# dyustc/CTC-Attention-Mispronunciation

Measured on AMD Instinct MI355X. Metric: phoneme-frames/sec joint CTC-attn decode, 41-phone vocab, higher is better.
Workload: dtype f32 -- reference width (operands with all 24 significand bits, fp32 accumulate; see `accuracy`: closer to a float64 evaluation than ATen's own fp32): the large time-batched contractions (conv0/conv1, BiLSTM and text input projections) run on the bf16 matrix cores as f32x6 = each fp32 operand as thre

## Files before the change

### ctc-attention-mispronunciation_amd/csrc/api.hip

```cpp
#include <stdarg.h>
#include <stdio.h>
#include <string.h>

#include <algorithm>
#include <cmath>
#include <memory>
#include <mutex>
#include <vector>

#include "mdd_internal.h"

namespace mdd {

static thread_local char g_err[512] = "";

void set_error(const char *fmt, ...) {
    va_list ap;
    va_start(ap, fmt);
    vsnprintf(g_err, sizeof(g_err), fmt, ap);
    va_end(ap);
}

struct DeviceGate {
    std::mutex mu;
// ... 266 lines not shown
    const ForwardPlan &p = m->plan;
    a.gx = m->gx.p; a.whh = lw.whh; a.hbuf = m->hbuf.p; a.cbuf = m->cbuf.p;
    a.H = m->cfg.hidden; a.packed = packed_whh(m->cfg);
    a.whh_split = lw.whh_s; a.hsplit = p.lstm == Lstm::StepX3 ? reinterpret_cast<unsigned short *>(m->hsplit.p) : nullptr;
    if (!p.gated) return launch_lstm_layer(a, st);
    info->launches = 1;
    unsigned short *hx = reinterpret_cast<unsigned short *>(m->hx.p);
    long long *stamps = m->sw.lstm_dbg && a.T > 100 ? reinterpret_cast<long long *>(m->hx.p + p.stamps_at) : nullptr;
    if (p.lstm == Lstm::X6) return launch_lstm_layer_x6(a, lw.whh_3, hx, m->sync_words.p, m->err_flag.p, st, stamps, m->sw.x6_redo_mask);
    if (p.lstm == Lstm::Granule) return launch_lstm_layer_granule(a, hx, m->sync_words.p, m->err_flag.p, st, stamps, m->sw.lstm_early);
    return launch_lstm_layer_f32(a, hx, m->sync_words.p, m->err_flag.p, st, stamps);
}

static int run_stage(mdd_model *m, int si, const float *x, int B, int T, const int64_t *x1, int L, float *logp,
                     hipStream_t st, Stage *info) {
    const mdd_config &c = m->cfg;
    const DecodeWeights &w = *m->weights;
    const int H = c.hidden, H2 = 2 * H, G2 = 8 * H, Tp = T / 2, Lp = L, nl = c.layers;
    const ForwardPlan &p = m->plan;
    const bool x3 = p.precision == 1, fused = p.conv != Conv::Separate;
    const size_t rows = (size_t)Tp * B, trows = (size_t)L * B;
    static thread_local char namebuf[32];
    Stage dummy; if (!info) info = &dummy;
    info->launches = 1; info->flops = 0.0;
    if (si == 0 && fused) {
        info->name = "conv_fused";
        info->flops = 2.0 * 9 * c.channels * (double)B * Tp * m->W2() * (c.channels + 6.0);
        if (p.conv == Conv::FusedX3)
            return launch_conv_fused(x, w.w_conv0, w.sc0, w.sh0, w.w_conv1_s, w.sc1, w.sh1, split_view(m->seq0_s, rows * m->rnn_in()),
                                     nullptr, B, T, m->raw_T, st);
        return launch_conv_fused3(x, w.w_conv0, w.sc0, w.sh0, w.w_conv1_3, w.sc1, w.sh1, reinterpret_cast<unsigned short *>(m->p3.p),
                                  m->taps ? m->seq0.p : nullptr, B, T, m->raw_T, st, p.conv == Conv::FusedX6Rowwise);
    }
    if (si == 1 && fused) { info->name = "conv1_in_fused"; info->launches = 0; return MDD_OK; }
    if (si == 0) { info->name = "conv0"; info->flops = 2.0 * 9 * c.channels * (double)B * T * m->W1();
        return launch_conv0(x, w.w_conv0, w.sc0, w.sh0, m->y0.p, B, T, c.feat, c.channels, st); }
    if (si == 1) { info->name = "conv1"; info->flops = 2.0 * 9 * c.channels * c.channels * (double)B * Tp * m->W2();
        return launch_conv1(m->y0.p, w.w_conv1t, w.sc1, w.sh1, x3 ? nullptr : m->seq0.p,
                            x3 ? split_view(m->seq0_s, rows * m->rnn_in()) : kNoSplit, B, T, m->W1(), c.channels, st); }
    si -= 2;
    if (si < 2 * nl) {
        const int n = si / 2;
        const int K = n == 0 ? m->rnn_in() : H2;
        if (si % 2 == 0) {
            snprintf(namebuf, sizeof(namebuf), "gemm_ih%d", n); info->name = namebuf;
            info->flops = 2.0 * (double)Tp * B * G2 * K;
            if (p.proj == Gemm::Bf16x3) {
                const SplitPtr in = n == 0 ? split_view(m->seq0_s, rows * K) : split_view(m->act_s[(n - 1) & 1], rows * K);
                return launch_gemm_bf16x3(in, w.rnn[n].wih_s, nullptr, m->gx.p, nullptr, Tp * B, G2, K, K, K, G2, 1, 0, 0, 0, st);
            }
            const float *in = n == 0 ? m->seq0.p : m->act[(n - 1) & 1].p;
            if (p.proj == Gemm::F32x6) {
                unsigned short *p3 = reinterpret_cast<unsigned short *>(m->p3.p);
                if (!(n == 0 && fused))
                    if (int rc = launch_split3(in, Tp * B, K, K, p3, st)) return rc;
                return launch_gemm_f32x6(p3, (size_t)Tp * B * K, w.rnn[n].wih_3, (size_t)G2 * K, nullptr, m->gx.p, Tp * B, G2, K, G2, st);
            }
            return launch_gemm_nt(in, w.rnn[n].wih, nullptr, m->gx.p, Tp * B, G2, K, K, K, G2, 1, 0, 0, 0, st);
        }
        snprintf(namebuf, sizeof(namebuf), "lstm%d", n); info->name = namebuf;
        info->launches = Tp; info->flops = 2.0 * 2 * (double)B * H * 4 * H * Tp;
        LstmStepArgs a;
        a.T = Tp; a.B = B; a.seqlen = m->tlen;
        if (n == nl - 1) {
            a.out = m->xraw.p; a.out_raw = m->xraw.p; a.oscale = nullptr; a.oshift = nullptr;
            a.out_split = x3 ? split_view(m->x_s, rows * H2) : kNoSplit;
        } else {
            a.out = x3 ? nullptr : m->act[n & 1].p; a.out_raw = m->taps ? m->tap_rnn[n].p : nullptr;
            a.out_split = x3 ? split_view(m->act_s[n & 1], rows * H2) : kNoSplit;
            a.oscale = w.rnn[n + 1].scale; a.oshift = w.rnn[n + 1].shift;
        }
        return run_lstm(m, w.rnn[n], a, st, info);
    }
    si -= 2 * nl;
    const LstmWeights &tw = w.rnn[nl];
    switch (si) {
    case 0:
        info->name = "embed";
        return launch_embed(w.emb, c.emb_rows, c.emb_dim, x1, B, L, x3 ? nullptr : m->embo.p,
                            x3 ? split_view(m->embo_s, trows * c.emb_dim) : kNoSplit, m->err_flag.p, st);
    case 1:
        info->name = "gemm_text"; info->flops = 2.0 * (double)L * B * G2 * c.emb_dim;
        if (p.proj == Gemm::Bf16x3) return launch_gemm_bf16x3(split_view(m->embo_s, trows * c.emb_dim), tw.wih_s, w.t_bias, m->gx.p, nullptr, L * B, G2,
                                                              c.emb_dim, c.emb_dim, c.emb_dim, G2, 1, 0, 0, 0, st);
        if (p.proj == Gemm::F32x6) {
            unsigned short *p3 = reinterpret_cast<unsigned short *>(m->p3.p);
            if (int rc = launch_split3(m->embo.p, L * B, c.emb_dim, c.emb_dim, p3, st)) return rc;
            return launch_gemm_f32x6(p3, (size_t)L * B * c.emb_dim, tw.wih_3, (size_t)G2 * c.emb_dim, w.t_bias, m->gx.p, L * B, G2, c.emb_dim, G2, st);
        }
        return launch_gemm_nt(m->embo.p, tw.wih, w.t_bias, m->gx.p, L * B, G2, c.emb_dim, c.emb_dim, c.emb_dim, G2, 1, 0, 0, 0, st);
    case 2: {
        info->name = "lstm_text"; info->launches = L; info->flops = 2.0 * 2 * (double)B * H * 4 * H * L;
        LstmStepArgs a;
        a.T = L; a.B = B; a.seqlen = m->llen;
        a.out = m->text.p; a.out_raw = m->text.p; a.oscale = nullptr; a.oshift = nullptr;
        a.out_split = x3 ? split_view(m->text_s, trows * H2) : kNoSplit;
        return run_lstm(m, tw, a, st, info);
    }
    case 3:
        info->name = "gemm_key"; info->flops = 2.0 * (double)L * B * H2 * H2;
        if (x3) {
            const SplitPtr ks = split_view(m->key_s, trows * H2);
            return launch_gemm_bf16x3(split_view(m->text_s, trows * H2), w.w_score_s, nullptr, nullptr, &ks, L * B, H2, H2, H2, H2, H2,
                                      1, 0, 0, 0, st);
        }
        return launch_gemm_nt(m->text.p, w.w_score, nullptr, m->key.p, L * B, H2, H2, H2, H2, H2, 1, 0, 0, 0, st);
    case 4:
        info->name = "gemm_score"; info->flops = 2.0 * (double)B * Tp * L * H2;
        if (x3) return launch_gemm_bf16x3(split_view(m->x_s, rows * H2), split_view(m->key_s, trows * H2), nullptr, m->S.p, nullptr, Tp, L,
                                          H2, B * H2, B * H2, Lp, B, H2, H2, (long)Tp * Lp, st);
        return launch_gemm_nt(m->xraw.p, m->key.p, nullptr, m->S.p, Tp, L, H2, B * H2, B * H2, Lp, B, H2, H2, (long)Tp * Lp, st);
    default:
        info->name = "attn_tail"; info->flops = 2.0 * (double)B * Tp * ((double)L * H2 + 2.0 * H2 * c.num_class);
        return launch_attn_tail(m->S.p, Lp, m->xraw.p, m->text.p, w.fscale, w.fshift, w.w_fc, w.w_fcp, logp, Tp, B, L, H2, c.num_class, st, m->llen);
    }
}

int device_gate_enter(int device, hipStream_t st, bool *held) {
    *held = false;
    hipStreamCaptureStatus cs = hipStreamCaptureStatusNone;
    if (st && hipStreamIsCapturing(st, &cs) == hipSuccess && cs != hipStreamCaptureStatusNone) return MDD_OK;
// ... 355 lines not shown
```

### ctc-attention-mispronunciation_amd/csrc/lstm_x6.hip

```cpp
#include "lstm_persist.h"
#include <type_traits>
#include <utility>

namespace mdd {

typedef __bf16 bf16x8 __attribute__((ext_vector_type(8)));

#define XSTAMP(i) do { if (DBG) { long long n_ = __builtin_readcyclecounter(); ph[i] += n_ - tst; tst = n_; } } while (0)

template <int N, typename F>
__device__ __forceinline__ void x6_static_for(F &&f) {
    if constexpr (N > 0) { x6_static_for<N - 1>(f); f(std::integral_constant<int, N - 1>{}); }
}

struct X6Args {
    const float *gx;
    const unsigned short *whh3;
    unsigned short *hx;
    unsigned int *sync;
    int *err_flag;
    float *out, *out_raw;
    const float *oscale, *oshift;
    int T, B, BGr;
    int force_mask;
    long long *dbg;
    const int *seqlen;
};

template <int H, int NBT, bool DBG = false>
__global__ __launch_bounds__(256, 1) void lstm_layer_x6_kernel(X6Args a) {
    extern __shared__ __attribute__((aligned(16))) unsigned char smem[];
    constexpr int NTH = 256, KS = H / 32, KH = KS / 2, RM = 4 * H / 16, NRT = RM / 16, UW = RM / 4;
    static_assert(NRT == 6 || NRT == 4, "H = 384 (six row tiles per member) or H = 256 (four)");
    constexpr int NT = NRT / 2;
    constexpr int CPM = UW / 8;
    constexpr bool SKEW = NBT >= 3;
    constexpr int CC = H / 8;
    constexpr int PLB = CC * 256;
    constexpr int PANB = 3 * PLB;
    constexpr int NLD = PANB / (NTH * 16);
    static_assert(PANB % (NTH * 16) == 0 && (NLD == 9 || NLD == 6), "a panel is whole passes of the workgroup");
    constexpr int NGB = NBT == 1 ? 2 : 1;
    constexpr int GXT = 16 * UW * 4;
    float *Os = reinterpret_cast<float *>(smem);
    float *Or = Os + 16 * UW;
    unsigned short *Og = reinterpret_cast<unsigned short *>(Or + 16 * UW);
    float *Gx = reinterpret_cast<float *>(Og + 3 * 3 * 16 * 8);
    unsigned char *Rw = reinterpret_cast<unsigned char *>(Gx + NBT * NGB * GXT);
    float *Px = reinterpret_cast<float *>(Rw + 2 * PANB);
    __shared__ int s_flag[3];
    const int tid = threadIdx.x, lane = tid & 63, wave = tid >> 6;
    const int li = lane & 15, kq = lane >> 4;
    const int w = blockIdx.x, xl = w & 7, jw = w >> 3;
    const int team = xl * 2 + (jw >> 4), member = jw & 15;
    const int d = team >> 3, g = team & 7;
    const int B = a.B, T = a.T;
    if (tid < 3) s_flag[tid] = 0;
    const int rh = wave >> 1, kh = wave & 1;

    bf16x8 wf[NT][KH][3];
#pragma unroll
    for (int t = 0; t < NT; t++) {
        const int rt = t < 2 ? rh * 2 + t : 4 + rh;
        const int row = member * RM + rt * 16 + li;
#pragma unroll
        for (int p = 0; p < 3; p++) {
            const unsigned short *wp = a.whh3 + ((size_t)(p * 2 + d) * 4 * H + row) * H + kq * 8 + kh * KH * 32;
#pragma unroll
            for (int j = 0; j < KH; j++) wf[t][j][p] = *reinterpret_cast<const bf16x8 *>(wp + j * 32);
        }
    }
    const int ot0 = kh == 0 ? rh * 2 : 4;
    const int widx = kh == 0 ? rh : 2;
    float osc[2], osh[2];
    const bool scaled = a.oscale != nullptr;
#pragma unroll
    for (int r = 0; r < 2; r++) {
        const int unit = member * UW + min(ot0 + r, NRT - 1) * 4 + kq;
        osc[r] = scaled ? a.oscale[d * H + unit] : 1.f;
        osh[r] = scaled ? a.oshift[d * H + unit] : 0.f;
    }
    float cst[2][NBT];
#pragma unroll
    for (int r = 0; r < 2; r++)
#pragma unroll
        for (int bt = 0; bt < NBT; bt++) cst[r][bt] = 0.f;
    int slen[NBT];
#pragma unroll
    for (int bt = 0; bt < NBT; bt++) {
        const int lb = bt * 16 + li, row = g * a.BGr + lb;
        slen[bt] = (a.seqlen && lb < a.BGr && row < B) ? a.seqlen[row] : T;
    }
    constexpr size_t tbytes = PANB;
    const size_t pbytes = (size_t)NBT * tbytes;
    unsigned char *hxb = reinterpret_cast<unsigned char *>(a.hx);
    unsigned int *abortf = a.sync + 16;
    long long ph[6] = {0, 0, 0, 0, 0, 0}, tst = DBG ? (long long)__builtin_readcyclecounter() : 0;

    const unsigned gx_lds = (unsigned)(unsigned long long)(lds_void_t *)Gx, rw_lds = (unsigned)(unsigned long long)(lds_void_t *)Rw;
// ... 29 lines not shown
#undef X6_G
#undef X6_G2
    };
    const unsigned char *const hx_team = hxb + (size_t)team * pbytes;
    auto hx_parity = [&](int sp) { return hx_team + (size_t)(sp & 1) * 16 * pbytes; };
    auto tag_word = [](int sp) -> unsigned { const unsigned ep = (unsigned)(sp % 3 + 1); return ((ep & 1u) << 14) | ((ep >> 1) << 30); };
    auto panel_stale = [&](int pb, int sp) -> bool {
        const unsigned e = tag_word(sp);
        unsigned bad = 0;
#pragma unroll
        for (int i = 0; i < NLD; i++) bad |= *reinterpret_cast<const unsigned *>(Rw + (size_t)pb * PANB + (size_t)(i * NTH + tid) * 16) ^ e;
        return (bad & 0x40004000u) != 0;
    };
    int fk = 0;
    auto wg_any = [&](bool v) -> bool {
        if (__any(v) && lane == 0) s_flag[fk] = 1;
        lds_barrier();
        const bool r = s_flag[fk] != 0;
        const int nx = fk == 2 ? 0 : fk + 1, n2 = nx == 2 ? 0 : nx + 1;
        if (tid == 0) s_flag[n2] = 0;
        fk = nx;
        return r;
    };
    int vslot = 0;
    auto post = [&](bool v) { if (__any(v) && lane == 0) s_flag[fk] = 1; };
    auto posted = [&] {
        vslot = fk;
        const int nx = fk == 2 ? 0 : fk + 1, n2 = nx == 2 ? 0 : nx + 1;
        if (tid == 0) s_flag[n2] = 0;
        fk = nx;
    };
    auto ensure_fresh = [&](int bt, int sp, int pb) -> bool {
        long long t0 = 0;
        int polls = 0;
        bool ok = true;
        for (;;) {
            request_sweep(hx_parity(sp), bt, pb);
            asm volatile("s_waitcnt vmcnt(0)" ::: "memory");
            lds_barrier();
            if ((++polls & 63) == 0) {
                bool giveup = false;
                if (t0 == 0) t0 = wall_clock64();
                if (tid == 0 && ((__hip_atomic_load(abortf, __ATOMIC_RELAXED, __HIP_MEMORY_SCOPE_AGENT) != 0) || (wall_clock64() - t0 > 200000000ll))) {
                    __hip_atomic_store(abortf, 1u, __ATOMIC_RELAXED, __HIP_MEMORY_SCOPE_AGENT); atomicExch(a.err_flag, 2); giveup = true;
                }
                if (wg_any(giveup)) { ok = false; break; }
            }
            if (!wg_any(panel_stale(pb, sp))) break;
        }
        if (DBG) ph[5] += polls;
        return ok;
    };
    const size_t slab = (size_t)B * 2 * H;
    const bool two_out = a.out_raw && a.out && a.out_raw != a.out;
    float *const out_main = a.out ? a.out : a.out_raw;
    auto tile_rows = [&](int bt) { const int nv = min(a.BGr, B - g * a.BGr) - bt * 16; return nv < 0 ? 0 : (nv > 16 ? 16 : nv); };

    auto products = [&](auto chk_, int pb, unsigned e, f32x4 *gsum, auto &&at_ks, auto &&pre) -> bool {
        constexpr bool CHK = decltype(chk_)::value;
        const unsigned char *fb = Rw + (size_t)pb * PANB + kq * 256 + li * 16 + kh * (KH * 1024);
        unsigned orall = 0u, andall = ~0u;
        if (CHK) {
            const unsigned char *ob = Rw + (size_t)pb * PANB + kq * 256 + li * 16 + (kh ^ 1) * (KH * 1024);
#pragma unroll
            for (int j = 0; j < KH; j++)
#pragma unroll
                for (int p = 0; p < 3; p++) { const unsigned v = *reinterpret_cast<const unsigned *>(ob + p * PLB + j * 1024); orall |= v; andall &= v; }
        }
        const f32x4 z = (f32x4){0.f, 0.f, 0.f, 0.f};
        f32x4 hh[NT], sm[NT];
#pragma unroll
        for (int t = 0; t < NT; t++) { hh[t] = z; sm[t] = z; }
        u32x4 fh[3][3];
#pragma unroll
        for (int p = 0; p < 3; p++) { fh[0][p] = *reinterpret_cast<const u32x4 *>(fb + p * PLB); fh[1][p] = *reinterpret_cast<const u32x4 *>(fb + p * PLB + 1024); }
        pre();
#pragma unroll
        for (int p = 0; p < 3; p++) {
            if (CHK) { orall |= fh[0][p][0]; andall &= fh[0][p][0]; }
            fh[0][p][0] &= 0xbfffbfffu;
        }
#pragma unroll
        for (int j = 0; j < KH; j++) {
            __builtin_amdgcn_sched_barrier(0x406);
            if (j + 2 < KH) {
#pragma unroll
                for (int p = 0; p < 3; p++) fh[(j + 2) % 3][p] = *reinterpret_cast<const u32x4 *>(fb + p * PLB + (j + 2) * 1024);
            }
            at_ks(j);
            if (j + 1 < KH) {
#pragma unroll
                for (int p = 0; p < 3; p++) {
                    if (CHK) { orall |= fh[(j + 1) % 3][p][0]; andall &= fh[(j + 1) % 3][p][0]; }
                    fh[(j + 1) % 3][p][0] &= 0xbfffbfffu;
                }
            }
            const bf16x8 bh = __builtin_bit_cast(bf16x8, fh[j % 3][0]), bm = __builtin_bit_cast(bf16x8, fh[j % 3][1]), bl = __builtin_bit_cast(bf16x8, fh[j % 3][2]);
#define X6_MF(acc, wp, bp) _Pragma("unroll") for (int t = 0; t < NT; t++) acc[t] = __builtin_amdgcn_mfma_f32_16x16x32_bf16(wf[t][j][wp], bp, acc[t], 0, 0, 0)
            X6_MF(sm, 1, bm); X6_MF(sm, 0, bl); X6_MF(sm, 2, bh); X6_MF(hh, 0, bh); X6_MF(sm, 0, bm); X6_MF(sm, 1, bh);
#undef X6_MF
        }
#pragma unroll
        for (int t = 0; t < NT; t++) gsum[t] = hh[t] + sm[t];
        return CHK && (((orall ^ e) | (andall ^ e)) & 0x40004000u) != 0;
    };
    auto px_at = [&](int buf, int tile, int half) -> float * { return Px + ((buf * 6 + tile) * 2 + half) * 256 + lane * 4; };
    auto send_partials = [&](auto role_, const f32x4 *gsum, int buf) {
        constexpr int ROLE = decltype(role_)::value;
#pragma unroll
        for (int t = 0; t < NT; t++) {
            const bool own = ROLE == 0 ? t < 2 : (ROLE == 1 && t == 2);
            if (!own) *reinterpret_cast<f32x4 *>(px_at(buf, t < 2 ? rh * 2 + t : 4 + rh, kh)) = gsum[t];
        }
    };

    auto cell1 = [&](auto role_, const f32x4 *gsum, int buf, auto bt_, int sc, bool on) {
        constexpr int ROLE = decltype(role_)::value;
        constexpr int bt = decltype(bt_)::value;
        const int t = d ? (T - 1 - sc) : sc;
        const unsigned tg = (unsigned)(sc % 3 + 1);
        const int lb = bt * 16 + li;
        const bool valid = lb < a.BGr && g * a.BGr + lb < B;
        const int gb = NBT == 1 ? (sc & 1) : 0;
#pragma unroll
        for (int r = 0; r < 2; r++) {
            const int rt = ot0 + r;
            f32x4 acc;
            if (ROLE == 0) acc = gsum[r] + *reinterpret_cast<const f32x4 *>(px_at(buf, rt, 1));
            else if (r == 0) acc = gsum[2] + *reinterpret_cast<const f32x4 *>(px_at(buf, 4, 0));
            else acc = *reinterpret_cast<const f32x4 *>(px_at(buf, 5, 0)) + *reinterpret_cast<const f32x4 *>(px_at(buf, 5, 1));
            const float4 gv = *reinterpret_cast<const float4 *>(Gx + (bt * NGB + gb) * GXT + (rt * 64 + lane) * 4);
            const float gi = acc[0] + gv.x, gf = acc[1] + gv.y, gg = acc[2] + gv.z, go = acc[3] + gv.w;
            const float ig = gate_sigmoid(gi), fg = gate_sigmoid(gf), cg = gate_tanh(gg), og = gate_sigmoid(go);
            const bool live = !(d && t >= slen[bt]);
            const float cn = fg * cst[r][bt] + ig * cg;
            const float hr_ = og * gate_tanh(cn);
            const float hn = (valid && live) ? hr_ : 0.f;
            cst[r][bt] = on ? (live ? cn : 0.f) : cst[r][bt];
            const int ul = rt * 4 + kq;
            Os[li * UW + ul] = scaled ? hn * osc[r] + osh[r] : hn;
            Or[li * UW + ul] = hn;
            const unsigned tagw = r == 0 ? ((kq == 0 ? (tg & 1u) : kq == 1 ? (tg >> 1) : 0u) << 14) : 0u;
            const float hs = (hn != hn) ? 1.5f : hn;
            const __bf16 b0 = (__bf16)hs;
            const float r1 = hs - (float)b0;
            const __bf16 b1 = (__bf16)r1, b2 = (__bf16)(r1 - (float)b1);
            unsigned short *og_ = Og + widx * (3 * 16 * 8) + li * 8 + r * 4 + kq;
            og_[0] = (unsigned short)(__builtin_bit_cast(unsigned short, b0) | tagw);
            og_[16 * 8] = (unsigned short)(__builtin_bit_cast(unsigned short, b1) | tagw);
            og_[2 * 16 * 8] = (unsigned short)(__builtin_bit_cast(unsigned short, b2) | tagw);
        }
    };
    auto cell2 = [&](auto bt_, const float *gxn, unsigned char *hxpub, float *outp, float *rawp, bool on) {
        constexpr int bt = decltype(bt_)::value;
        if (NBT >= 2) load_gx(bt, 0, gxn);
        {
            const int prow = lane & 15, pp = lane >> 4;
            const __amdgpu_buffer_rsrc_t drs = __builtin_amdgcn_make_buffer_rsrc(hxpub + (size_t)bt * tbytes, 0, (int)tbytes, 0x00020000);
            const u32x4 pv = *reinterpret_cast<const u32x4 *>(Og + widx * (3 * 16 * 8) + ((pp < 3 ? pp : 0) * 16 + prow) * 8);
            const unsigned off = (pp < 3 && on) ? (unsigned)(pp * PLB + ((member * CPM + (ot0 >> 1)) * 16 + prow) * 16) : 0xffffffffu;
            __builtin_amdgcn_raw_buffer_store_b128(pv, drs, off, 0, 16 );
        }
        {
            const int nr = tile_rows(bt);
            const int rr = min(lane & 15, max(nr - 1, 0)), piece = lane >> 4;
            const bool mine = piece < 2 && nr > 0 && on;
            const int rt = ot0 + (piece & 1);
            const unsigned el = (unsigned)((g * a.BGr + bt * 16 + rr) * 2 * H + d * H + member * UW + rt * 4);
            const int lo = rr * UW + rt * 4;
            const u32x4 v = *reinterpret_cast<const u32x4 *>(Os + lo);
            const __amdgpu_buffer_rsrc_t rs_ = __builtin_amdgcn_make_buffer_rsrc(outp, 0, (int)(slab * 4), 0x00020000);
            __builtin_amdgcn_raw_buffer_store_b128(v, rs_, mine ? el * 4u : 0xffffffffu, 0, 0);
            const u32x4 v2 = *reinterpret_cast<const u32x4 *>(Or + lo);
            const __amdgpu_buffer_rsrc_t rs2 = __builtin_amdgcn_make_buffer_rsrc(rawp, 0, (int)(slab * 4), 0x00020000);
            __builtin_amdgcn_raw_buffer_store_b128(v2, rs2, (mine && two_out) ? el * 4u : 0xffffffffu, 0, 0);
        }
    };

    auto run = [&](auto role_) {
        constexpr int ROLE = decltype(role_)::value;
        constexpr bool OWNER = ROLE == 0 || (ROLE == 1 && NRT == 6);
        const std::integral_constant<bool, ROLE == 2> chk_{};
#pragma unroll
        for (int i = 0; i < 2 * NLD; i++) *reinterpret_cast<u32x4 *>(Rw + (size_t)(i * NTH + tid) * 16) = (u32x4){0u, 0u, 0u, 0u};
        if constexpr (OWNER) x6_static_for<NBT>([&](auto bt_) { load_gx(decltype(bt_)::value, 0, gx_at(d ? (T - 1) : 0)); });
        asm volatile("s_waitcnt vmcnt(0)" ::: "memory");
        lds_barrier();
        f32x4 gP[NT];
#pragma unroll
        for (int t = 0; t < NT; t++) gP[t] = (f32x4){0.f, 0.f, 0.f, 0.f};
        int pc = 0;
        bool dead = false, have_v = false;
        auto redo = [&](int btv, int sv, int pbv, int pxb) {
            asm volatile("s_waitcnt vmcnt(0)" ::: "memory");
            if (!ensure_fresh(btv, sv - 1, pbv)) { dead = true; return; }
            products(std::false_type{}, pbv, 0u, gP, [](int) {}, [] {});
            send_partials(role_, gP, pxb);
            lds_barrier();
            if (DBG) ph[5] += 1000;
        };
        float *const raw_main = two_out ? a.out_raw : out_main;
        auto t_of = [&](int st) { return d ? (T - 1 - st) : st; };
        for (int s = 0; s < T && !dead; s++) {
            const int sp_ = max(s - 1, 0), sn_ = min(s + 1, T - 1);
            const float *const gx_s = gx_at(t_of(s)), *const gx_n = gx_at(t_of(sn_));
            float *const out_s = out_main + (size_t)t_of(s) * slab, *const out_p = out_main + (size_t)t_of(sp_) * slab;
            float *const raw_s = raw_main + (size_t)t_of(s) * slab, *const raw_p = raw_main + (size_t)t_of(sp_) * slab;
            unsigned char *const hx_s = const_cast<unsigned char *>(hx_parity(s)), *const hx_p = const_cast<unsigned char *>(hx_parity(s - 1));
            auto phase = [&](auto bt_) {
                constexpr int bt = decltype(bt_)::value;
                constexpr int nbt = bt + 1 < NBT ? bt + 1 : 0, pbt = bt > 0 ? bt - 1 : NBT - 1;
                const int ns = bt + 1 < NBT ? s : s + 1, psv = bt > 0 ? s : s - 1;
                const int pb = pc & 1;
                ++pc;
                f32x4 gs[NT];
                if (NBT == 1) {
                    if (s >= 1) {
                        asm volatile("s_waitcnt vmcnt(0)" ::: "memory");
                        if (!ensure_fresh(bt, s - 1, pb)) { dead = true; return; }
                    }
                    XSTAMP(0);
                    products(std::false_type{}, pb, 0u, gs, [&](int j) { if (OWNER && j == 0) load_gx(bt, (s + 1) & 1, gx_n); }, [] {});
                    XSTAMP(1);
                    send_partials(role_, gs, 0);
                    asm volatile("s_waitcnt vmcnt(0)" ::: "memory");
                    lds_barrier();
                    XSTAMP(2);
                    if constexpr (OWNER) { cell1(role_, gs, 0, bt_, s, true); XSTAMP(3); cell2(bt_, gx_n, hx_s, out_s, raw_s, true); }
                    XSTAMP(4);
                    return;
                }
                constexpr int RQJ = SKEW ? 0 : KH - 1;
                const bool stale = products(chk_, pb, tag_word(s + 2), gs, [&](int j) {
                    if (j == RQJ) request_sweep(hx_parity(ns - 1), nbt, pb ^ 1);
                    if constexpr (SKEW && OWNER) {
                        if (j == 0) cell1(role_, gP, (pc & 1), std::integral_constant<int, pbt>{}, max(psv, 0), psv >= 0);
                        if (j == 1) { if (bt > 0) cell2(std::integral_constant<int, pbt>{}, gx_n, hx_s, out_s, raw_s, true); else cell2(std::integral_constant<int, pbt>{}, gx_s, hx_p, out_p, raw_p, psv >= 0); }
                    }
                }, [&] {
                    if constexpr (SKEW) { if (have_v && s_flag[vslot] != 0) redo(pbt, psv, pb ^ 1, pc & 1); }
                }) && s >= 1;
                const bool forced = a.force_mask >= 0 && s >= 1 && (pc & a.force_mask) == 0;
                XSTAMP(1);
                send_partials(role_, gs, (pc & 1) ^ 1);
                if constexpr (SKEW) {
                    post(stale || forced);
                    if constexpr (OWNER) wait_vmcnt(3); else asm volatile("s_waitcnt vmcnt(0)" ::: "memory");
                    lds_barrier();
                    posted();
                    have_v = true;
                    XSTAMP(2);
                } else {
                    const bool again = wg_any(stale || forced);
                    XSTAMP(2);
                    if (again) {
                        asm volatile("s_waitcnt vmcnt(0)" ::: "memory");
                        if (!ensure_fresh(bt, s - 1, pb)) { dead = true; return; }
                        products(std::false_type{}, pb, 0u, gs, [](int) {}, [] {});
                        send_partials(role_, gs, (pc & 1) ^ 1);
                        lds_barrier();
                        if (DBG) ph[5] += 1000;
                    }
                }
                if (SKEW) {
#pragma unroll
                    for (int t = 0; t < NT; t++) gP[t] = gs[t];
                } else {
                    if constexpr (OWNER) cell1(role_, gs, (pc & 1) ^ 1, bt_, s, true);
                    XSTAMP(3);
                    asm volatile("s_waitcnt vmcnt(0)" ::: "memory");
                    lds_barrier();
                    if constexpr (OWNER) cell2(bt_, gx_n, hx_s, out_s, raw_s, true);
                    XSTAMP(4);
                }
                XSTAMP(0);
            };
            x6_static_for<NBT>([&](auto bt_) { if (!dead) phase(bt_); });
        }
        if constexpr (SKEW) {
            if (!dead && have_v && s_flag[vslot] != 0) redo(NBT - 1, T - 1, (pc & 1) ^ 1, (pc & 1) ^ 1);
            if constexpr (OWNER) {
                if (!dead) {
                    cell1(role_, gP, (pc & 1) ^ 1, std::integral_constant<int, NBT - 1>{}, T - 1, true);
                    cell2(std::integral_constant<int, NBT - 1>{}, gx_at(t_of(T - 1)), const_cast<unsigned char *>(hx_parity(T - 1)), out_main + (size_t)t_of(T - 1) * slab, raw_main + (size_t)t_of(T - 1) * slab, true);
                }
            }
        }
    };
    if (kh == 0) run(std::integral_constant<int, 0>{});
    else if (rh == 0) run(std::integral_constant<int, 1>{});
    else run(std::integral_constant<int, 2>{});
    if (DBG && tid == ((blockIdx.x >> 3) & 3) * 64)
        for (int i = 0; i < 6; i++) a.dbg[blockIdx.x * 6 + i] = ph[i];
}

static size_t x6_smem(int H, int NBT) {
    const int UW = H / 16;
    return (size_t)16 * UW * 4 * 2 + (size_t)3 * 3 * 16 * 8 * 2 + (size_t)NBT * (NBT == 1 ? 2 : 1) * 16 * UW * 16 + (size_t)2 * 3 * (H / 8) * 256 + (size_t)2 * 6 * 2 * 1024;
}

template <int H, int NBT, bool DBG = false>
static int launch_x6_t(const X6Args &a, hipStream_t st) {
    if (int rc = launch_zero_fill(a.sync, 32 * sizeof(unsigned int), st)) return rc;
    if (int rc = launch_zero_fill(a.hx, (size_t)2 * 16 * NBT * 3 * (H / 8) * 256, st)) return rc;
    hipLaunchKernelGGL((lstm_layer_x6_kernel<H, NBT, DBG>), dim3(kPersistGrid), dim3(256), x6_smem(H, NBT), st, a);
    MDD_LAUNCH_CHECK();
    return MDD_OK;
}

template <int H, int N>
static constexpr bool x6_built() {
#ifdef MDD_X6_DEV
    return H == 384 && N <= 4;
#else
    return true;
#endif
}
template <int H, int N>
static int launch_x6_pick(const X6Args &a, hipStream_t st) {
    if constexpr (!x6_built<H, N>()) { set_error("persistent x6 lstm: H=%d with %d tiles per team is not in this development build", H, N); return MDD_ERR_ARG; }
    else {
        if constexpr (H == 384) { if (a.dbg) return launch_x6_t<H, N, true>(a, st); }
        return launch_x6_t<H, N>(a, st);
    }
}

int launch_lstm_layer_x6(const LstmStepArgs &s, const unsigned short *whh3, unsigned short *hx, unsigned int *sync, int *err_flag, hipStream_t st,
                         long long *stamps, int force_mask) {
    X6Args a;
    a.gx = s.gx; a.whh3 = whh3; a.hx = hx; a.sync = sync; a.err_flag = err_flag;
    a.out = s.out; a.out_raw = s.out_raw; a.oscale = s.oscale; a.oshift = s.oscale ? s.oshift : nullptr;
    a.T = s.T; a.B = s.B; a.BGr = (s.B + 7) / 8; a.seqlen = s.seqlen;
    a.force_mask = force_mask;
    const int nbt = (a.BGr + 15) / 16;
    a.dbg = stamps;
    if (s.out_split.hi || s.gates_save || (!a.out && !a.out_raw) || !whh3) { set_error("persistent x6 lstm: fp32 outputs, inference only"); return MDD_ERR_ARG; }
    if (nbt < 1 || nbt > 8) { set_error("persistent x6 lstm: B=%d needs %d row tiles per team (max 8)", s.B, nbt); return MDD_ERR_ARG; }
#define X6_CASE(H_, N_) case N_: return launch_x6_pick<H_, N_>(a, st)
    if (s.H == 384) switch (nbt) { X6_CASE(384, 1); X6_CASE(384, 2); X6_CASE(384, 3); X6_CASE(384, 4); X6_CASE(384, 5); X6_CASE(384, 6); X6_CASE(384, 7); X6_CASE(384, 8); }
    if (s.H == 256) switch (nbt) { X6_CASE(256, 1); X6_CASE(256, 2); X6_CASE(256, 3); X6_CASE(256, 4); X6_CASE(256, 5); X6_CASE(256, 6); X6_CASE(256, 7); X6_CASE(256, 8); }
#undef X6_CASE
    set_error("persistent x6 lstm: unsupported H=%d", s.H);
    return MDD_ERR_ARG;
}

template <int H, int N>
static int x6_attr() {
    if constexpr (x6_built<H, N>()) {
        MDD_HIP_CHECK(hipFuncSetAttribute((const void *)lstm_layer_x6_kernel<H, N>, hipFuncAttributeMaxDynamicSharedMemorySize, 156 * 1024));
        if constexpr (H == 384) MDD_HIP_CHECK(hipFuncSetAttribute((const void *)lstm_layer_x6_kernel<H, N, true>, hipFuncAttributeMaxDynamicSharedMemorySize, 156 * 1024));
    }
    return MDD_OK;
}

int init_lstm_x6_attributes() {
#define XATTR(H, N) if (int rc = x6_attr<H, N>()) return rc
    XATTR(384, 1); XATTR(384, 2); XATTR(384, 3); XATTR(384, 4); XATTR(384, 5); XATTR(384, 6); XATTR(384, 7); XATTR(384, 8);
    XATTR(256, 1); XATTR(256, 2); XATTR(256, 3); XATTR(256, 4); XATTR(256, 5); XATTR(256, 6); XATTR(256, 7); XATTR(256, 8);
#undef XATTR
    return MDD_OK;
}

int persistent_x6_grid_fits(int n_cu) {
    if (n_cu < kPersistGrid) return 0;
    int per_cu = 0;
    constexpr int N = x6_built<384, 8>() ? 8 : 4;
    if (hipOccupancyMaxActiveBlocksPerMultiprocessor(&per_cu, (const void *)lstm_layer_x6_kernel<384, N>, 256, x6_smem(384, N)) != hipSuccess) return 0;
    return per_cu >= 1 ? 1 : 0;
}

}
```

### ctc-attention-mispronunciation_amd/csrc/mdd_internal.h

```cpp
#pragma once
#include <hip/hip_runtime.h>
#include <stdint.h>

#include <map>
#include <string>
#include <utility>
#include <vector>

#include "../../include/mdd_hip.h"
#include "plan.h"

namespace mdd {

void set_error(const char *fmt, ...);

#define MDD_HIP_CHECK(expr)                                                                     \
    do {                                                                                        \
        hipError_t e_ = (expr);                                                                 \
        if (e_ != hipSuccess) {                                                                 \
            mdd::set_error("%s failed: %s (%s:%d)", #expr, hipGetErrorString(e_), __FILE__, __LINE__); \
            return MDD_ERR_HIP;                                                                 \
        }                                                                                       \
    } while (0)

// ... 19 lines not shown
    }
};
using DeviceBuf = DeviceArray<float>;

struct SplitPtr { unsigned short *hi, *lo; };

int launch_gemm_nt(const float *A, const float *W, const float *bias, float *C, int M, int N, int K, int lda, int ldw,
                   int ldc, int batch, long sA, long sW, long sC, hipStream_t st);

int launch_gemm_f32(bool ta, bool tb, const float *A, const float *B, const float *bias, float *C, int M, int N, int K, int lda, int ldb,
                    int ldc, int batch, long sA, long sB, long sC, bool accumulate, hipStream_t st, int ksplit = 0);

int launch_gemm_bf16x3(const SplitPtr &A, const SplitPtr &W, const float *bias, float *C, const SplitPtr *Csplit, int M, int N,
                       int K, int lda, int ldw, int ldc, int batch, long sA, long sW, long sC, hipStream_t st);
int init_gemm_attributes();
int launch_split(const float *x, size_t n, const SplitPtr &out, hipStream_t st);
int launch_unsplit(const SplitPtr &in, size_t n, float *x, hipStream_t st);
int launch_split3(const float *x, int rows, int K, int ld, unsigned short *planes, hipStream_t st);
int launch_gemm_f32x6(const unsigned short *A3, size_t a_plane, const unsigned short *W3, size_t w_plane, const float *bias, float *C, int M, int N, int K,
                      int ldc, hipStream_t st, long long *stamps = nullptr);
int init_gemm_x6_attributes();

int launch_stack_skip(const float *raw, int B, int T_raw, int D, int right, int skip, int n_down, float *out,
                      hipStream_t st);
int launch_conv0(const float *x, const float *w, const float *scale, const float *shift, float *y0, int B, int T, int F,
                 int ch, hipStream_t st);
int launch_conv1(const float *y0, const float *w_t, const float *scale, const float *shift, float *seq, SplitPtr seq_split, int B,
                 int T, int W1, int ch, hipStream_t st);

int launch_conv_fused(const float *x, const float *w0, const float *sc0, const float *sh0, SplitPtr w1, const float *sc1,
                      const float *sh1, SplitPtr out, float *out_f32, int B, int T, int Traw, hipStream_t st);
int launch_conv_fused3(const float *x, const float *w0, const float *sc0, const float *sh0, const unsigned short *w1_3, const float *sc1,
                       const float *sh1, unsigned short *out3, float *out_f32, int B, int T, int Traw, hipStream_t st,
                       bool rowwise = false);
int init_conv_attributes();

struct LstmStepArgs {
    const float *gx;
    const float *whh;
    float *hbuf;
    float *cbuf;
    float *out;
    SplitPtr out_split;
    float *out_raw;
    const float *oscale;
    const float *oshift;
    int T, B, H;
    SplitPtr whh_split;
    unsigned short *hsplit;
    int packed;
    float *gates_save = nullptr;
    float *c_save = nullptr;
    const int *seqlen = nullptr;
};
int launch_lstm_layer(const LstmStepArgs &a, hipStream_t st);

int launch_embed(const float *table, int rows, int E, const int64_t *ids, int B, int L, float *out, SplitPtr out_split,
                 int *err_flag, hipStream_t st);
int launch_attn_tail(const float *S, int Lp, const float *X, const float *V, const float *fscale, const float *fshift,
                     const float *wfc, const float *wfcp, float *logp, int Tp, int B, int L, int H2, int C, hipStream_t st,
                     const int *llen = nullptr);

int init_kernel_attributes();
int init_ctc_attributes();
int init_lstm_attributes();
int init_granule_attributes();
int persistent_grid_fits(int n_cu);
int launch_lstm_layer_granule(const LstmStepArgs &s, unsigned short *hx, unsigned int *sync, int *err_flag, hipStream_t st,
                              long long *stamps = nullptr, bool early = false);
int launch_zero_fill(void *p, size_t n, hipStream_t st);
int launch_lstm_layer_f32(const LstmStepArgs &s, unsigned short *hx, unsigned int *sync, int *err_flag, hipStream_t st, long long *stamps);
int init_lstm_f32_attributes();
int persistent_f32_grid_fits(int n_cu);
int launch_lstm_layer_x6(const LstmStepArgs &s, const unsigned short *whh3, unsigned short *hx, unsigned int *sync, int *err_flag, hipStream_t st,
                         long long *stamps, int force_mask);
int init_lstm_x6_attributes();
int persistent_x6_grid_fits(int n_cu);
size_t lstm_bwd_granule_hx_bytes(int H);
int launch_lstm_bwd_granule(const float *dout, const float *gates, const float *cst, SplitPtr whhT, float *dg, int T, int B, int H, unsigned short *hx,
                            unsigned int *sync, int *err_flag, hipStream_t st);
int device_gate_enter(int device, hipStream_t st, bool *held);
int device_gate_leave(int device, hipStream_t st, bool held, int rc);

}
```

### ctc-attention-mispronunciation_amd/csrc/plan.h

```cpp
#pragma once
#include <stddef.h>
#include <stdlib.h>
#include <string.h>

#include "../../include/mdd_hip.h"

namespace mdd {

struct Switches {
    int precision = 2;
    bool graph = true;
    bool lstm_step = false;
    bool lstm_x3 = false;
    bool x6_off = false;
    bool x6_force = false;
    bool conv_rowwise = false;
    bool lstm_dbg = false;
    bool lstm_early = false;
    int x6_redo_mask = -1;
};

inline Switches read_switches() {
    Switches s;
    auto is = [](const char *e, const char *v) { return e && !strcmp(e, v); };
    const char *e = getenv("MDD_PRECISION");
    if (is(e, "f32") || is(e, "0")) s.precision = 0;
    if (is(e, "bf16x3") || is(e, "1")) s.precision = 1;
    e = getenv("MDD_GRAPH");
    s.graph = !(e && e[0] == '0');
    e = getenv("MDD_LSTM");
    s.lstm_step = is(e, "step");
    s.lstm_x3 = is(e, "x3");
    e = getenv("MDD_LSTM_X6");
    s.x6_off = e && e[0] == '0';
    s.x6_force = e && e[0] == 'f';
    s.conv_rowwise = is(getenv("MDD_CONV"), "rowwise");
    s.lstm_dbg = getenv("MDD_LSTM_DBG") != nullptr;
    s.lstm_early = getenv("MDD_LSTM_EARLY") != nullptr;
    e = getenv("MDD_X6_FORCE_REDO");
    const int n = e ? atoi(e) : 0;
    if (n > 0 && (n & (n - 1)) == 0) s.x6_redo_mask = n - 1;
    return s;
}

struct DeviceFit { bool granule, f32, x6; };

inline int conv_out(int w) { return (w + 2 - 3) / 2 + 1; }
inline int rnn_in(const mdd_config &c) { return c.channels * conv_out(conv_out(c.feat)); }

inline bool packed_whh(const mdd_config &c) { return c.hidden == 384 || c.hidden == 256; }

inline int granule_bg(int B) { const int r = (B + 15) / 16; return (r + 15) / 16 * 16; }
inline size_t lstm_x6_hx_bytes(int H, int B) { const int bgr = (B + 7) / 8, nbt = (bgr + 15) / 16; return (size_t)2 * 16 * nbt * 3 * (H / 8) * 256; }
static constexpr int kPersistMaxB = 1024;

enum class Conv { Separate, FusedX3, FusedX6, FusedX6Rowwise };
enum class Gemm { Nt, Bf16x3, F32x6 };
enum class Lstm { X6, F32, Granule, StepX3, StepPacked, Step };

struct ForwardPlan {
    int precision;
    Conv conv;
    Gemm proj;
    Lstm lstm;
    bool gated;
    size_t hx_floats;
    size_t stamps_at;
};

inline ForwardPlan plan_forward(const mdd_config &c, int precision, const Switches &sw, const DeviceFit &fit, int B) {
    const int H = c.hidden, K0 = rnn_in(c);
    const bool packed = packed_whh(c);
    const bool x3 = precision == 1 && packed && K0 % 32 == 0 && c.emb_dim % 32 == 0;
    const bool x6 = precision == 2 && K0 % 32 == 0 && (2 * H) % 32 == 0 && c.emb_dim % 32 == 0;
    ForwardPlan p{};
    p.precision = x3 ? 1 : x6 ? 2 : 0;
    if ((x3 || x6) && c.feat == 243 && c.channels == 32) p.conv = x3 ? Conv::FusedX3 : sw.conv_rowwise ? Conv::FusedX6Rowwise : Conv::FusedX6;
    else p.conv = Conv::Separate;
    p.proj = x3 ? Gemm::Bf16x3 : x6 ? Gemm::F32x6 : Gemm::Nt;
    const bool persist = fit.granule && !sw.lstm_step && !sw.lstm_x3 && packed && B <= kPersistMaxB && (x3 || fit.f32);
    const bool lx6 = x6 && persist && fit.x6 && !sw.x6_off && (sw.x6_force || H == 384 || B <= 128);
    if (lx6) p.lstm = Lstm::X6;
    else if (persist) p.lstm = x3 ? Lstm::Granule : Lstm::F32;
    else if (x3 && sw.lstm_x3) p.lstm = Lstm::StepX3;
    else p.lstm = packed ? Lstm::StepPacked : Lstm::Step;
    p.gated = persist;
    if (persist) {
        const size_t granules = (size_t)2 * 32 * granule_bg(B) * H * 2, planes = lstm_x6_hx_bytes(H, B) / 4;
        p.stamps_at = lx6 ? planes : granules;
        p.hx_floats = (lx6 && planes > granules ? planes : granules) + 64 + 256 * 6 * 2;
    }
    return p;
}

}
```

Baseline: 4.327 million.

## Emit bf16x3 split planes directly from persistent x6 LSTM, skip split3 pass

```diff
diff --git a/ctc-attention-mispronunciation_amd/csrc/api.hip b/ctc-attention-mispronunciation_amd/csrc/api.hip
--- a/ctc-attention-mispronunciation_amd/csrc/api.hip
+++ b/ctc-attention-mispronunciation_amd/csrc/api.hip
@@ -342,7 +342,7 @@
             const float *in = n == 0 ? m->seq0.p : m->act[(n - 1) & 1].p;
             if (p.proj == Gemm::F32x6) {
                 unsigned short *p3 = reinterpret_cast<unsigned short *>(m->p3.p);
-                if (!(n == 0 && fused))
+                if (!(n == 0 && fused) && !(n >= 1 && p.planes_out))
                     if (int rc = launch_split3(in, Tp * B, K, K, p3, st)) return rc;
                 return launch_gemm_f32x6(p3, (size_t)Tp * B * K, w.rnn[n].wih_3, (size_t)G2 * K, nullptr, m->gx.p, Tp * B, G2, K, G2, st);
             }
@@ -356,7 +356,10 @@
             a.out = m->xraw.p; a.out_raw = m->xraw.p; a.oscale = nullptr; a.oshift = nullptr;
             a.out_split = x3 ? split_view(m->x_s, rows * H2) : kNoSplit;
         } else {
-            a.out = x3 ? nullptr : m->act[n & 1].p; a.out_raw = m->taps ? m->tap_rnn[n].p : nullptr;
+            a.out = x3 || p.planes_out ? nullptr : m->act[n & 1].p; a.out_raw = m->taps ? m->tap_rnn[n].p : nullptr;
+            if (p.planes_out) {
+                a.out_planes = reinterpret_cast<unsigned short *>(m->p3.p); a.out_planes_stride = rows * H2;
+            }
             a.out_split = x3 ? split_view(m->act_s[n & 1], rows * H2) : kNoSplit;
             a.oscale = w.rnn[n + 1].scale; a.oshift = w.rnn[n + 1].shift;
         }
diff --git a/ctc-attention-mispronunciation_amd/csrc/lstm_x6.hip b/ctc-attention-mispronunciation_amd/csrc/lstm_x6.hip
--- a/ctc-attention-mispronunciation_amd/csrc/lstm_x6.hip
+++ b/ctc-attention-mispronunciation_amd/csrc/lstm_x6.hip
@@ -25,6 +25,9 @@
     int force_mask;
     long long *dbg;
     const int *seqlen;
+    unsigned short *planes;
+    size_t plane_stride;
+    int rows;
 };
 
 template <int H, int NBT, bool DBG = false>
@@ -43,8 +46,8 @@
     constexpr int NGB = NBT == 1 ? 2 : 1;
     constexpr int GXT = 16 * UW * 4;
     float *Os = reinterpret_cast<float *>(smem);
-    float *Or = Os + 16 * UW;
-    unsigned short *Og = reinterpret_cast<unsigned short *>(Or + 16 * UW);
+    float *Or = Os + 2 * 16 * UW;
+    unsigned short *Og = reinterpret_cast<unsigned short *>(Or + 2 * 16 * UW);
     float *Gx = reinterpret_cast<float *>(Og + 3 * 3 * 16 * 8);
     unsigned char *Rw = reinterpret_cast<unsigned char *>(Gx + NBT * NGB * GXT);
     float *Px = reinterpret_cast<float *>(Rw + 2 * PANB);
@@ -180,8 +183,8 @@
         return ok;
     };
     const size_t slab = (size_t)B * 2 * H;
-    const bool two_out = a.out_raw && a.out && a.out_raw != a.out;
-    float *const out_main = a.out ? a.out : a.out_raw;
+    float *const out_main = a.out ? a.out : (a.planes ? nullptr : a.out_raw);
+    float *const out_raw2 = (a.out_raw && a.out_raw != out_main) ? a.out_raw : nullptr;
     auto tile_rows = [&](int bt) { const int nv = min(a.BGr, B - g * a.BGr) - bt * 16; return nv < 0 ? 0 : (nv > 16 ? 16 : nv); };
 
     auto products = [&](auto chk_, int pb, unsigned e, f32x4 *gsum, auto &&at_ks, auto &&pre) -> bool {
@@ -242,7 +245,7 @@
         }
     };
 
-    auto cell1 = [&](auto role_, const f32x4 *gsum, int buf, auto bt_, int sc, bool on) {
+    auto cell1 = [&](auto role_, const f32x4 *gsum, int buf, auto bt_, int sc, bool on, int ob) {
         constexpr int ROLE = decltype(role_)::value;
         constexpr int bt = decltype(bt_)::value;
         const int t = d ? (T - 1 - sc) : sc;
@@ -266,8 +269,8 @@
             const float hn = (valid && live) ? hr_ : 0.f;
             cst[r][bt] = on ? (live ? cn : 0.f) : cst[r][bt];
             const int ul = rt * 4 + kq;
-            Os[li * UW + ul] = scaled ? hn * osc[r] + osh[r] : hn;
-            Or[li * UW + ul] = hn;
+            Os[ob * (16 * UW) + li * UW + ul] = scaled ? hn * osc[r] + osh[r] : hn;
+            Or[ob * (16 * UW) + li * UW + ul] = hn;
             const unsigned tagw = r == 0 ? ((kq == 0 ? (tg & 1u) : kq == 1 ? (tg >> 1) : 0u) << 14) : 0u;
             const float hs = (hn != hn) ? 1.5f : hn;
             const __bf16 b0 = (__bf16)hs;
@@ -279,7 +282,7 @@
             og_[2 * 16 * 8] = (unsigned short)(__builtin_bit_cast(unsigned short, b2) | tagw);
         }
     };
-    auto cell2 = [&](auto bt_, const float *gxn, unsigned char *hxpub, float *outp, float *rawp, bool on) {
+    auto cell2 = [&](auto bt_, const float *gxn, unsigned char *hxpub, bool on) {
         constexpr int bt = decltype(bt_)::value;
         if (NBT >= 2) load_gx(bt, 0, gxn);
         {
@@ -289,19 +292,52 @@
             const unsigned off = (pp < 3 && on) ? (unsigned)(pp * PLB + ((member * CPM + (ot0 >> 1)) * 16 + prow) * 16) : 0xffffffffu;
             __builtin_amdgcn_raw_buffer_store_b128(pv, drs, off, 0, 16 );
         }
-        {
-            const int nr = tile_rows(bt);
-            const int rr = min(lane & 15, max(nr - 1, 0)), piece = lane >> 4;
-            const bool mine = piece < 2 && nr > 0 && on;
-            const int rt = ot0 + (piece & 1);
-            const unsigned el = (unsigned)((g * a.BGr + bt * 16 + rr) * 2 * H + d * H + member * UW + rt * 4);
-            const int lo = rr * UW + rt * 4;
-            const u32x4 v = *reinterpret_cast<const u32x4 *>(Os + lo);
-            const __amdgpu_buffer_rsrc_t rs_ = __builtin_amdgcn_make_buffer_rsrc(outp, 0, (int)(slab * 4), 0x00020000);
-            __builtin_amdgcn_raw_buffer_store_b128(v, rs_, mine ? el * 4u : 0xffffffffu, 0, 0);
-            const u32x4 v2 = *reinterpret_cast<const u32x4 *>(Or + lo);
-            const __amdgpu_buffer_rsrc_t rs2 = __builtin_amdgcn_make_buffer_rsrc(rawp, 0, (int)(slab * 4), 0x00020000);
-            __builtin_amdgcn_raw_buffer_store_b128(v2, rs2, (mine && two_out) ? el * 4u : 0xffffffffu, 0, 0);
+    };
+    constexpr int NFS = (16 * (UW / 4) + 63) / 64;
+    const int n_out = (a.planes ? 3 : 0) + (out_main ? NFS : 0) + (out_raw2 ? NFS : 0);
+    auto emit = [&](auto bt_, int st, int ob, bool on) {
+        constexpr int bt = decltype(bt_)::value;
+        const int t = d ? (T - 1 - max(st, 0)) : max(st, 0);
+        const int nr = on ? tile_rows(bt) : 0;
+        const float *os = Os + ob * (16 * UW), *orw = Or + ob * (16 * UW);
+        if (a.planes) {
+            const int cc = min(kq, CPM - 1);
+            const bool mine = kq < CPM && li < nr;
+            const f32x4 v0 = *reinterpret_cast<const f32x4 *>(os + li * UW + cc * 8), v1 = *reinterpret_cast<const f32x4 *>(os + li * UW + cc * 8 + 4);
+            typedef float f32x2 __attribute__((ext_vector_type(2)));
+            typedef __bf16 bf16x2 __attribute__((ext_vector_type(2)));
+            u32x4 p0, p1, p2;
+#pragma unroll
+            for (int i = 0; i < 4; i++) {
+                const f32x2 x = i < 2 ? (f32x2){v0[(i & 1) * 2], v0[(i & 1) * 2 + 1]} : (f32x2){v1[(i & 1) * 2], v1[(i & 1) * 2 + 1]};
+                const unsigned w0 = __builtin_bit_cast(unsigned, __builtin_convertvector(x, bf16x2));
+                const f32x2 r1 = x - (f32x2){__builtin_bit_cast(float, w0 << 16), __builtin_bit_cast(float, w0 & 0xffff0000u)};
+                const unsigned w1 = __builtin_bit_cast(unsigned, __builtin_convertvector(r1, bf16x2));
+                const f32x2 r2 = r1 - (f32x2){__builtin_bit_cast(float, w1 << 16), __builtin_bit_cast(float, w1 & 0xffff0000u)};
+                p0[i] = w0; p1[i] = w1; p2[i] = __builtin_bit_cast(unsigned, __builtin_convertvector(r2, bf16x2));
+            }
+            const int k = d * H + member * UW + cc * 8;
+            const unsigned row = (unsigned)(t * B + g * a.BGr + bt * 16 + li);
+            const unsigned off = mine ? (((unsigned)(k >> 5) * (unsigned)a.rows + row) * 32u + (unsigned)(k & 31)) * 2u : 0xffffffffu;
+            const int pbytes_ = (int)((unsigned)a.rows * (unsigned)(2 * H) * 2u);
+            __builtin_amdgcn_raw_buffer_store_b128(p0, __builtin_amdgcn_make_buffer_rsrc(a.planes, 0, pbytes_, 0x00020000), off, 0, 0);
+            __builtin_amdgcn_raw_buffer_store_b128(p1, __builtin_amdgcn_make_buffer_rsrc(a.planes + a.plane_stride, 0, pbytes_, 0x00020000), off, 0, 0);
+            __builtin_amdgcn_raw_buffer_store_b128(p2, __builtin_amdgcn_make_buffer_rsrc(a.planes + 2 * a.plane_stride, 0, pbytes_, 0x00020000), off, 0, 0);
+        }
+#pragma unroll
+        for (int i = 0; i < NFS; i++) {
+            const int piece = i * 4 + kq;
+            const bool mine = piece < UW / 4 && li < nr;
+            const int lo = li * UW + min(piece, UW / 4 - 1) * 4;
+            const unsigned off = mine ? (unsigned)((g * a.BGr + bt * 16 + li) * 2 * H + d * H + member * UW + piece * 4) * 4u : 0xffffffffu;
+            if (out_main) {
+                const u32x4 v = *reinterpret_cast<const u32x4 *>(os + lo);
+                __builtin_amdgcn_raw_buffer_store_b128(v, __builtin_amdgcn_make_buffer_rsrc(out_main + (size_t)t * slab, 0, (int)(slab * 4), 0x00020000), off, 0, 0);
+            }
+            if (out_raw2) {
+                const u32x4 v = *reinterpret_cast<const u32x4 *>(orw + lo);
+                __builtin_amdgcn_raw_buffer_store_b128(v, __builtin_amdgcn_make_buffer_rsrc(out_raw2 + (size_t)t * slab, 0, (int)(slab * 4), 0x00020000), off, 0, 0);
+            }
         }
     };
 
@@ -327,13 +363,10 @@
             lds_barrier();
             if (DBG) ph[5] += 1000;
         };
-        float *const raw_main = two_out ? a.out_raw : out_main;
         auto t_of = [&](int st) { return d ? (T - 1 - st) : st; };
         for (int s = 0; s < T && !dead; s++) {
-            const int sp_ = max(s - 1, 0), sn_ = min(s + 1, T - 1);
+            const int sn_ = min(s + 1, T - 1);
             const float *const gx_s = gx_at(t_of(s)), *const gx_n = gx_at(t_of(sn_));
-            float *const out_s = out_main + (size_t)t_of(s) * slab, *const out_p = out_main + (size_t)t_of(sp_) * slab;
-            float *const raw_s = raw_main + (size_t)t_of(s) * slab, *const raw_p = raw_main + (size_t)t_of(sp_) * slab;
             unsigned char *const hx_s = const_cast<unsigned char *>(hx_parity(s)), *const hx_p = const_cast<unsigned char *>(hx_parity(s - 1));
             auto phase = [&](auto bt_) {
                 constexpr int bt = decltype(bt_)::value;
@@ -354,7 +387,8 @@
                     asm volatile("s_waitcnt vmcnt(0)" ::: "memory");
                     lds_barrier();
                     XSTAMP(2);
-                    if constexpr (OWNER) { cell1(role_, gs, 0, bt_, s, true); XSTAMP(3); cell2(bt_, gx_n, hx_s, out_s, raw_s, true); }
+                    if constexpr (OWNER) { cell1(role_, gs, 0, bt_, s, true, s & 1); XSTAMP(3); cell2(bt_, gx_n, hx_s, true); }
+                    if constexpr (ROLE == 2) emit(bt_, s - 1, (s & 1) ^ 1, s >= 1);
                     XSTAMP(4);
                     return;
                 }
@@ -362,8 +396,8 @@
                 const bool stale = products(chk_, pb, tag_word(s + 2), gs, [&](int j) {
                     if (j == RQJ) request_sweep(hx_parity(ns - 1), nbt, pb ^ 1);
                     if constexpr (SKEW && OWNER) {
-                        if (j == 0) cell1(role_, gP, (pc & 1), std::integral_constant<int, pbt>{}, max(psv, 0), psv >= 0);
-                        if (j == 1) { if (bt > 0) cell2(std::integral_constant<int, pbt>{}, gx_n, hx_s, out_s, raw_s, true); else cell2(std::integral_constant<int, pbt>{}, gx_s, hx_p, out_p, raw_p, psv >= 0); }
+                        if (j == 0) cell1(role_, gP, (pc & 1), std::integral_constant<int, pbt>{}, max(psv, 0), psv >= 0, pc & 1);
+                        if (j == 1) { if (bt > 0) cell2(std::integral_constant<int, pbt>{}, gx_n, hx_s, true); else cell2(std::integral_constant<int, pbt>{}, gx_s, hx_p, psv >= 0); }
                     }
                 }, [&] {
                     if constexpr (SKEW) { if (have_v && s_flag[vslot] != 0) redo(pbt, psv, pb ^ 1, pc & 1); }
@@ -373,7 +407,13 @@
                 send_partials(role_, gs, (pc & 1) ^ 1);
                 if constexpr (SKEW) {
                     post(stale || forced);
-                    if constexpr (OWNER) wait_vmcnt(3); else asm volatile("s_waitcnt vmcnt(0)" ::: "memory");
+                    if constexpr (ROLE == 2) {
+                        constexpr int ebt = (bt + NBT - 2) % NBT;
+                        const int es = bt >= 2 ? s : s - 1;
+                        emit(std::integral_constant<int, ebt>{}, es, (pc & 1) ^ 1, es >= 0);
+                        XSTAMP(3);
+                    }
+                    if constexpr (OWNER) wait_vmcnt(1); else if constexpr (ROLE == 2) { if (n_out == 3) wait_vmcnt(3); else wait_vmcnt(n_out); } else asm volatile("s_waitcnt vmcnt(0)" ::: "memory");
                     lds_barrier();
                     posted();
                     have_v = true;
@@ -394,11 +434,12 @@
 #pragma unroll
                     for (int t = 0; t < NT; t++) gP[t] = gs[t];
                 } else {
-                    if constexpr (OWNER) cell1(role_, gs, (pc & 1) ^ 1, bt_, s, true);
+                    if constexpr (OWNER) cell1(role_, gs, (pc & 1) ^ 1, bt_, s, true, pc & 1);
+                    if constexpr (ROLE == 2) emit(std::integral_constant<int, pbt>{}, psv, (pc & 1) ^ 1, psv >= 0);
                     XSTAMP(3);
-                    asm volatile("s_waitcnt vmcnt(0)" ::: "memory");
+                    if constexpr (ROLE == 2) wait_vmcnt(n_out); else asm volatile("s_waitcnt vmcnt(0)" ::: "memory");
                     lds_barrier();
-                    if constexpr (OWNER) cell2(bt_, gx_n, hx_s, out_s, raw_s, true);
+                    if constexpr (OWNER) cell2(bt_, gx_n, hx_s, true);
                     XSTAMP(4);
                 }
                 XSTAMP(0);
@@ -407,11 +448,23 @@
         }
         if constexpr (SKEW) {
             if (!dead && have_v && s_flag[vslot] != 0) redo(NBT - 1, T - 1, (pc & 1) ^ 1, (pc & 1) ^ 1);
-            if constexpr (OWNER) {
-                if (!dead) {
-                    cell1(role_, gP, (pc & 1) ^ 1, std::integral_constant<int, NBT - 1>{}, T - 1, true);
-                    cell2(std::integral_constant<int, NBT - 1>{}, gx_at(t_of(T - 1)), const_cast<unsigned char *>(hx_parity(T - 1)), out_main + (size_t)t_of(T - 1) * slab, raw_main + (size_t)t_of(T - 1) * slab, true);
+            if (!dead) {
+                if constexpr (OWNER) {
+                    cell1(role_, gP, (pc & 1) ^ 1, std::integral_constant<int, NBT - 1>{}, T - 1, true, (pc & 1) ^ 1);
+                    cell2(std::integral_constant<int, NBT - 1>{}, gx_at(t_of(T - 1)), const_cast<unsigned char *>(hx_parity(T - 1)), true);
                 }
+                if constexpr (ROLE == 2) emit(std::integral_constant<int, NBT - 2>{}, T - 1, pc & 1, true);
+                lds_barrier();
+                if constexpr (ROLE == 2) emit(std::integral_constant<int, NBT - 1>{}, T - 1, (pc & 1) ^ 1, true);
+            }
+        }
+        if constexpr (NBT == 2) {
+            if constexpr (ROLE == 2) { if (!dead) emit(std::integral_constant<int, 1>{}, T - 1, pc & 1, true); }
+        }
+        if constexpr (NBT == 1) {
+            if (!dead) {
+                lds_barrier();
+                if constexpr (ROLE == 2) emit(std::integral_constant<int, 0>{}, T - 1, (T - 1) & 1, true);
             }
         }
     };
@@ -424,7 +477,7 @@
 
 static size_t x6_smem(int H, int NBT) {
     const int UW = H / 16;
-    return (size_t)16 * UW * 4 * 2 + (size_t)3 * 3 * 16 * 8 * 2 + (size_t)NBT * (NBT == 1 ? 2 : 1) * 16 * UW * 16 + (size_t)2 * 3 * (H / 8) * 256 + (size_t)2 * 6 * 2 * 1024;
+    return (size_t)2 * 16 * UW * 4 * 2 + (size_t)3 * 3 * 16 * 8 * 2 + (size_t)NBT * (NBT == 1 ? 2 : 1) * 16 * UW * 16 + (size_t)2 * 3 * (H / 8) * 256 + (size_t)2 * 6 * 2 * 1024;
 }
 
 template <int H, int NBT, bool DBG = false>
@@ -462,7 +515,9 @@
     a.force_mask = force_mask;
     const int nbt = (a.BGr + 15) / 16;
     a.dbg = stamps;
-    if (s.out_split.hi || s.gates_save || (!a.out && !a.out_raw) || !whh3) { set_error("persistent x6 lstm: fp32 outputs, inference only"); return MDD_ERR_ARG; }
+    a.planes = s.out_planes; a.plane_stride = s.out_planes_stride; a.rows = s.T * s.B;
+    if (a.planes && (double)a.rows * (2 * s.H) * 2 >= 4294967296.0) { set_error("persistent x6 lstm: a plane of %d x %d elements is beyond the 32-bit store offsets", a.rows, 2 * s.H); return MDD_ERR_ARG; }
+    if (s.out_split.hi || s.gates_save || (!a.out && !a.out_raw && !a.planes) || !whh3) { set_error("persistent x6 lstm: fp32 outputs, inference only"); return MDD_ERR_ARG; }
     if (nbt < 1 || nbt > 8) { set_error("persistent x6 lstm: B=%d needs %d row tiles per team (max 8)", s.B, nbt); return MDD_ERR_ARG; }
 #define X6_CASE(H_, N_) case N_: return launch_x6_pick<H_, N_>(a, st)
     if (s.H == 384) switch (nbt) { X6_CASE(384, 1); X6_CASE(384, 2); X6_CASE(384, 3); X6_CASE(384, 4); X6_CASE(384, 5); X6_CASE(384, 6); X6_CASE(384, 7); X6_CASE(384, 8); }
diff --git a/ctc-attention-mispronunciation_amd/csrc/mdd_internal.h b/ctc-attention-mispronunciation_amd/csrc/mdd_internal.h
--- a/ctc-attention-mispronunciation_amd/csrc/mdd_internal.h
+++ b/ctc-attention-mispronunciation_amd/csrc/mdd_internal.h
@@ -95,6 +95,8 @@
     float *gates_save = nullptr;
     float *c_save = nullptr;
     const int *seqlen = nullptr;
+    unsigned short *out_planes = nullptr;
+    size_t out_planes_stride = 0;
 };
 int launch_lstm_layer(const LstmStepArgs &a, hipStream_t st);
 
diff --git a/ctc-attention-mispronunciation_amd/csrc/plan.h b/ctc-attention-mispronunciation_amd/csrc/plan.h
--- a/ctc-attention-mispronunciation_amd/csrc/plan.h
+++ b/ctc-attention-mispronunciation_amd/csrc/plan.h
@@ -18,6 +18,7 @@
     bool lstm_dbg = false;
     bool lstm_early = false;
     int x6_redo_mask = -1;
+    bool x6_out_fp32 = false;
 };
 
 inline Switches read_switches() {
@@ -40,6 +41,7 @@
     e = getenv("MDD_X6_FORCE_REDO");
     const int n = e ? atoi(e) : 0;
     if (n > 0 && (n & (n - 1)) == 0) s.x6_redo_mask = n - 1;
+    s.x6_out_fp32 = is(getenv("MDD_X6_OUT"), "fp32");
     return s;
 }
 
@@ -66,6 +68,7 @@
     bool gated;
     size_t hx_floats;
     size_t stamps_at;
+    bool planes_out;
 };
 
 inline ForwardPlan plan_forward(const mdd_config &c, int precision, const Switches &sw, const DeviceFit &fit, int B) {
@@ -85,6 +88,7 @@
     else if (x3 && sw.lstm_x3) p.lstm = Lstm::StepX3;
     else p.lstm = packed ? Lstm::StepPacked : Lstm::Step;
     p.gated = persist;
+    p.planes_out = p.proj == Gemm::F32x6 && lx6 && !sw.x6_out_fp32;
     if (persist) {
         const size_t granules = (size_t)2 * 32 * granule_bg(B) * H * 2, planes = lstm_x6_hx_bytes(H, B) / 4;
         p.stamps_at = lx6 ? planes : granules;
```

Result: faster. 4.403 million (median of 6 runs) (+1.7%).
